# masa-ue/SVDD

Measured on AMD Instinct MI355X. Metric: decoded sequences/sec (whole node), L=200 M=10 128-step SVDD-MC, higher is better.
Workload: dtype f32; 1 GPU; DNA enhancer SVDD-MC, batch=256/GPU, L=200, M=10, 128 steps (BASELINE.json configs[1]); dilated-CNN backbone 3.3M params + ConvGRU value net; global_batch=256, rng=philox

## Files before the change

### include/svdd_hip.h

```cpp
#ifndef SVDD_HIP_H
#define SVDD_HIP_H

#include <stdint.h>

#ifdef __cplusplus
extern "C" {
#endif

#define SVDD_VOCAB 5
#define SVDD_MASK 4
#define SVDD_MAX_M 1024

enum {
  SVDD_OK = 0,
  SVDD_E_ARG = -1,
  SVDD_E_LAUNCH = -2,
  SVDD_E_NODEVICE = -3
};

enum {
  SVDD_LAYOUT_BLV = 0,
  SVDD_LAYOUT_BVL = 1
};

// ... 109 lines not shown
int svdd_gru_set_mode(int mode);

int svdd_epilogue_ln_f32(const float* y, const float* bias, const float* f_prev, const float* tb,
                         const float* gamma, const float* beta, float* f_out, float* hn, int64_t rows,
                         int channels, int act, void* stream);

int svdd_conv1d_cl_f32(const float* x, const float* wpack, float* y, int n, int L, int cin, int cout,
                       int taps, int dilation, const float* bias, const float* f_prev, int act,
                       const float* tb, const float* gamma, const float* beta, float* hn, void* stream);
int svdd_conv1d_set_dynamic(int on);

int svdd_conv_tower_f32(const float* onehot, const float* tiles, const float* bias, float* out, int n, int L,
                        int nlayers, int residual_mask, const int32_t* count, void* stream);

int svdd_set_backbone_packing(int full);

int svdd_set_tower_version(int v);

int svdd_candidate_windows(const uint8_t* cand, const uint8_t* x, int B, int L, int M, int margin, int32_t* win,
                           int32_t* flags, void* stream);
int svdd_conv_tower_windows_f32(const float* onehot, const float* tiles, const float* bias, const int32_t* win,
                                const float* parent_out, float* out, int n, int L, int M, int nlayers,
                                int residual_mask, const int32_t* live_idx, const int32_t* count, void* stream);

int svdd_backbone_cnn_f32(const uint8_t* x, const float* table0, const float* tiles, const float* vec,
                          const float* w2, float* out, int n, int L, int nlayers, const int* dilations,
                          const int32_t* count, const int32_t* row_idx, int out_scatter, void* stream);
int svdd_backbone_cnn_save_f32(const uint8_t* x, const float* table0, const float* tiles, const float* vec, const float* w2,
                               float* out, int n, int L, int nlayers, const int* dilations, float* xhat, float* rstd,
                               unsigned long long* mask, void* stream);
int svdd_backbone_cnn_grad_f32(const float* dlogits, const float* tiles_bwd, const float* gamma, const float* w2,
                               const float* table0, const float* xhat, const float* rstd, const unsigned long long* mask,
                               float* dx, int n, int L, int nlayers, const int* dilations, void* stream);
int svdd_backbone_incr_f32(const uint8_t* x, const float* table0, const float* tiles, const float* vec, const float* w2,
                           float* out, int n, int L, int nlayers, const int* dilations, int lead, float* planes,
                           uint8_t* x_prev, int32_t* items, unsigned long long* stat, int first, int max_item, void* on_stream);
int svdd_backbone_incr2_f32(const uint8_t* x, const float* table0, const float* tiles, const float* vec, const float* w2,
                            float* out, int n, int L, int nlayers, const int* dilations, int lead, float* planes,
                            uint8_t* x_prev, int32_t* items, unsigned long long* stat, int first, int max_item,
                            int32_t* order, int32_t* order_count, void* on_stream);
int svdd_backbone_incr_set_residency(int wg_per_cu);
int svdd_backbone_set_workspace(void* ws, long long bytes);
int svdd_backbone_split_status(int* err);

enum { SVDD_PREC_F32 = 0, SVDD_PREC_F16X3 = 1, SVDD_PREC_BF16X3 = 2, SVDD_PREC_F16 = 3, SVDD_PREC_BF16 = 4 };

int svdd_backbone_cnn_lp(const uint8_t* x, const float* table0, const void* tiles, const float* vec,
                         const float* lscale, const float* w2, float* out, int n, int L, int nlayers,
                         const int* dilations, int prec, const int32_t* count, const int32_t* row_idx, int out_scatter,
                         void* stream);

int svdd_conv_tower_lp(const uint8_t* tok, const void* tiles, const float* bias, const float* inv, void* out,
                       int n, int L, int nlayers, int residual_mask, const int32_t* count, int prec, void* stream);
int svdd_conv_tower_windows_lp(const uint8_t* cand, const void* tiles, const float* bias, const float* inv,
                               const int32_t* win, const void* parent_out, void* out, int n, int L, int M,
                               int nlayers, int residual_mask, const int32_t* live_idx, const int32_t* count,
                               int prec, void* stream);

int svdd_gru_bidir_lp(const float* x, const void* x16, const void* wpack, const float* bpack, const float* inv,
                      float* out, int n, int L, const int32_t* count, int prec, void* stream);

int svdd_value_tail_lp(const float* h_fwd, const float* h_bwd, const void* w1pack, const float* b1,
                       const float* w_eff, const float* b_eff, float inv, float* out, int n, int L, int n_tasks,
                       const int32_t* count, int prec, void* stream);
// ... 69 lines not shown
```

### svdd_amd/_lib.py

```python
import ctypes
import os
import subprocess

_HERE = os.path.dirname(os.path.abspath(__file__))
CSRC = os.path.join(_HERE, "csrc")
SO_PATH = os.environ.get("SVDD_HIP_LIB") or os.path.join(CSRC, "libsvdd_hip.so")
ABI_VERSION = 17

OK, E_ARG, E_LAUNCH, E_NODEVICE = 0, -1, -2, -3
LAYOUT_BLV, LAYOUT_BVL = 0, 1
RNG_REPLAY, RNG_PHILOX = 0, 1
SELECT_ARGMAX, SELECT_MULTINOMIAL = 0, 1
TARGET_MEAN, TARGET_LOGMEANEXP = 0, 1
EVOLVE_GLOBAL, EVOLVE_ROW = 0, 1
ATTR_GRADIENT, ATTR_TIMES_INPUT = 0, 1
PRECISIONS = {"f32": 0, "f16x3": 1, "bf16x3": 2, "f16": 3, "bf16": 4}
MAX_M = 1024

OPT_FORCE_EXACT, OPT_MSPLIT, OPT_SELECT_ONE_ROW, OPT_BACKBONE_LP_VERSION, OPT_TRUNK_GEMM_VERSION = 0, 1, 2, 3, 4
OPT_CAND_ROW_STRIDE, OPT_TRUNK_PLANES_F32, OPT_BACKBONE_SPLIT, OPT_SELECT_BATCHES = 5, 6, 7, 8


class SvddRng(ctypes.Structure):
    _fields_ = [("kind", ctypes.c_int32), ("step", ctypes.c_uint32), ("uniforms", ctypes.c_void_p),
# ... 72 lines not shown
    "svdd_backbone_split_status": (pi32,),
    "svdd_backbone_cnn_save_f32": (vp, vp, vp, vp, vp, vp, i32, i32, i32, pi32, vp, vp, vp, STREAM),
    "svdd_backbone_cnn_grad_f32": (vp, vp, vp, vp, vp, vp, vp, vp, vp, i32, i32, i32, pi32, STREAM),
    "svdd_dps_probs": (vp, vp, i32, i32, vp, STREAM),
    "svdd_dps_probs_bwd": (vp, vp, vp, i32, i32, vp, vp, STREAM),
    "svdd_dps_guided_q": (vp, vp, vp, vp, f32, f32, f32, i32, i32, vp, STREAM),
    "svdd_reward_stem_f32": (vp, vp, vp, vp, i32, i32, i32, STREAM),
    "svdd_reward_stem_bwd_f32": (vp, vp, vp, i32, i32, i32, STREAM),
    "svdd_conv1d_cl_gated_f32": (vp, vp, vp, i32, i32, i32, i32, i32, i32, vp, vp, STREAM),
    "svdd_reward_tail_grad_f32": (vp, vp, vp, vp, vp, vp, vp, f32, i32, i32, vp, vp, STREAM),
    "svdd_sum_gate_f32": (vp, vp, vp, vp, i64, STREAM),
    "svdd_gru_bidir_train2_f32": (vp, vp, vp, vp, vp, vp, i32, i32, STREAM),
    "svdd_gru_bidir_bwd2_f32": (vp, vp, vp, vp, vp, vp, vp, i32, i32, STREAM),
    "svdd_classifier_propose": (vp, i32, vp, vp, f32, f32, f32, i32, i32, RNG, vp, vp, vp, STREAM),
    "svdd_elbo_mask": (vp, i32, i32, i32, f64, RNG, vp, vp, vp, vp, vp, vp, STREAM),
    "svdd_elbo_nll": (vp, i32, vp, vp, vp, i32, i32, i32, vp, vp, vp, vp, STREAM),
    "svdd_refine_remask": (vp, vp, vp, vp, vp, f32, i32, i32, RNG, vp, vp, vp, vp, vp, vp, vp),
    "svdd_value_target": (vp, vp, i32, i32, i32, i32, f32, vp, vp, vp, vp),
    "svdd_ism_mutants": (vp, vp, vp, i32, i32, i32, vp, vp, vp, vp),
    "svdd_ism_fold": (vp, vp, vp, vp, vp, vp, i32, i32, i32, i32, i32, vp, vp, vp, vp, vp),
    "svdd_evolve_apply": (vp, vp, vp, i32, i32, i32, vp, vp, vp, vp, vp, vp, vp, vp, vp, vp, vp, vp),
    "svdd_attr_path": (vp, vp, i32, vp, i32, i32, i32, i32, i32, i32, vp, vp, vp),
    "svdd_attr_fold": (vp, f32, vp, vp, vp, i32, i32, i32, i32, i32, i32, i32, vp, vp, vp, vp),
}
EXPORTS = tuple(SIGNATURES)


def build(force=False):
    import glob
    srcs = sorted(glob.glob(os.path.join(CSRC, "*.hip")) + glob.glob(os.path.join(CSRC, "*.h")) + [os.path.join(CSRC, "Makefile")])
    srcs.append(os.path.join(os.path.dirname(_HERE), "include", "svdd_hip.h"))
    if os.environ.get("SVDD_HIP_LIB"):
        return SO_PATH
    stale = not os.path.exists(SO_PATH) or os.path.getmtime(SO_PATH) < max(os.path.getmtime(f) for f in srcs)
    if force or stale:
        subprocess.check_call(["make", "-C", CSRC, "-B", "-j", str(min(8, os.cpu_count() or 1))])
    return SO_PATH


_lib = None


def lib():
    global _lib
    if _lib is not None:
        return _lib
# ... 112 lines not shown
```

### svdd_amd/csrc/svdd_nets.hip

```cpp
#include "svdd_host.h"

namespace {

typedef float f32x4 __attribute__((ext_vector_type(4)));

__device__ __forceinline__ float wave_sum(float v) {
#pragma unroll
  for (int off = 32; off > 0; off >>= 1) v += __shfl_xor(v, off, 64);
  return v;
}


constexpr int H = 64;
constexpr int HPAD = H + 4;

__device__ __forceinline__ float sigmoid_fast(float a) {
  return __builtin_amdgcn_rcpf(1.0f + __builtin_amdgcn_exp2f(-1.44269504088896f * a));
}
__device__ __forceinline__ float tanh_fast(float a) {
  return 1.0f - 2.0f * __builtin_amdgcn_rcpf(1.0f + __builtin_amdgcn_exp2f(2.88539008177793f * a));
}

template <bool BOTH>
__global__ __launch_bounds__(BOTH ? 512 : 256) void gru_bidir_kernel(const float* __restrict__ x, const float* __restrict__ wpack,
// ... 1163 lines not shown

__global__ __launch_bounds__(256) void candidate_windows_kernel(const uint8_t* __restrict__ cand, const uint8_t* __restrict__ x,
                                                               int n, int L, int M, int margin, int* __restrict__ win,
                                                               int* __restrict__ flags) {
  const int c = blockIdx.x * 4 + (threadIdx.x >> 6);
  if (c >= n) return;
  const int lane = threadIdx.x & 63;
  const uint8_t* cp = cand + (size_t)c * L;
  const uint8_t* xp = x + (size_t)(c / M) * L;
  int lo = 1 << 30, hi = -1;
  for (int l = lane; l < L; l += 64)
    if (cp[l] != xp[l]) { lo = min(lo, l); hi = max(hi, l); }
#pragma unroll
  for (int off = 32; off > 0; off >>= 1) { lo = min(lo, __shfl_xor(lo, off, 64)); hi = max(hi, __shfl_xor(hi, off, 64)); }
  if (lane == 0) {
    int w0 = 0, w1 = 0;
    if (hi >= 0) {
      w0 = max(0, lo - margin) & ~15;
      w1 = min((L + 15) & ~15, (hi + margin + 1 + 15) & ~15);
    }
    win[2 * c] = w0; win[2 * c + 1] = w1;
    if (flags) flags[c] = (w1 - w0) >> 4;
  }
}


struct BackboneArgs {
  const uint8_t* x;
  const float* table0;
  const float* tiles;
  const float* vec;
  const float* w2;
  float* out;
  int n, L, spt, nl;
  int dil[BB_MAXL];
  const int* count;
  const int* row_idx;
  int out_scatter;
  int auto_spt, ncu;
  SvddTilePlan plan;
  float* planes;
  int planes_P;
};

struct BackboneSave {
  float* xhat;
// ... 435 lines not shown
    const float* wv = a.w2 + v * BB_C;
    float sm = a.w2[5 * BB_C + v];
#pragma unroll 8
    for (int k = 0; k < BB_C; ++k) sm += hr[k] * wv[k];
    const int64_t sq = (a.row_idx && a.out_scatter) ? (int64_t)a.row_idx[seq0 + q] : (int64_t)(seq0 + q);
    a.out[(sq * L + pos) * 5 + v] = sm;
  }
}
#undef BB_OWN

constexpr int SEG_SLOTS = 7;

struct BackboneSegArgs {
  const uint8_t* x;
  const float* table0;
  const float* tiles;
  const float* vec;
  float* planes;
  const int* items;
  int n, L, layer;
  const int* order;
  const int* order_count;
  int order_stride;
};

template <int SLOTS = SEG_SLOTS>
__global__ __launch_bounds__(256) void backbone_worklist_kernel(const uint8_t* __restrict__ x, uint8_t* __restrict__ x_prev, int n,
                                                                int L, int P, int max_item, int* __restrict__ items,
                                                                unsigned long long* __restrict__ stat) {
  const int row = blockIdx.x * 4 + (threadIdx.x >> 6);
  if (row >= n) return;
  const int lane = threadIdx.x & 63;
  const uint8_t* xn = x + (size_t)row * L;
  uint8_t* xp = x_prev + (size_t)row * L;
  int changed = 0;
  for (int q = 0; q < 4; ++q) {
    const int l = lane + 64 * q;
    if (l < L && xn[l] != xp[l]) { changed |= 1 << q; xp[l] = xn[l]; }
  }
  int mine = 0;
  for (int k = 1; k <= P; ++k) {
    const int reach = 4 + 4 * k;
    int m = 0;
    for (int q = 0; q < 4; ++q)
      if (changed >> q & 1) {
        const int l = lane + 64 * q;
        const int tlo = max(0, l - reach) >> 4, thi = min(L - 1, l + reach) >> 4;
        m |= ((2 << thi) - 1) & ~((1 << tlo) - 1);
      }
#pragma unroll
    for (int off = 32; off > 0; off >>= 1) m |= __shfl_xor(m, off, 64);
    if (lane == k - 1) mine = m;
  }
  if (lane >= P) return;
  int* it = items + ((size_t)lane * n + row) * SLOTS;
  int cnt = 0;
  for (int t = 0; t < TW_RT;) {
    if (!(mine >> t & 1)) { ++t; continue; }
    int len = 1;
    while (len < max_item && t + len < TW_RT && (mine >> (t + len) & 1)) ++len;
    it[cnt++] = t | len << 8;
// ... 72 lines not shown
    if ((int)blockIdx.x >= a.order_count[a.layer - 1]) return;
    const unsigned ent = (unsigned)__builtin_amdgcn_readfirstlane(a.order[(size_t)(a.layer - 1) * a.order_stride + blockIdx.x]);
    item = (int)(ent & 0xFFFFu);
    seq = (int)(ent >> 16);
  } else {
    item = __builtin_amdgcn_readfirstlane(a.items[(size_t)(a.layer - 1) * a.n * SEG_SLOTS + blockIdx.x]);
    seq = blockIdx.x / SEG_SLOTS;
  }
  const int nown = min(item >> 8, NC);
  if (nown == 0) return;
  const int t0 = item & 255;
  const int tid = threadIdx.x, lane = tid & 63;
  const int cg = __builtin_amdgcn_readfirstlane(tid >> 6);
  const int j = lane & 15, g = lane >> 4;
  const int col0 = 32 * cg + j;
  const int L = a.L;
  const int r0 = 16 * (t0 - 1);
  const size_t pl_stride = (size_t)a.n * TW_ROWS * BB_C;
  float* pl0 = a.planes + (size_t)seq * TW_ROWS * BB_C;
  const int cl = a.layer - 1;
#define SEG_LIVE(S) ((S) <= nown + 1)

  f32x4 f[NS][2], acc[NS][2];
  if (a.layer == 1) {
    for (int e = tid; e < ROWS + 8; e += 256) {
      const int p = r0 - 4 + e;
      toks[e] = (p >= 0 && p < L) ? (int)a.x[(size_t)seq * L + p] : -1;
    }
    __syncthreads();
#pragma unroll
    for (int ct = 0; ct < 2; ++ct) {
      const int col = col0 + 16 * ct;
      const float b0 = a.vec[col];
#pragma unroll
      for (int s = 0; s < NS; ++s) {
        if (!SEG_LIVE(s)) continue;
#pragma unroll
        for (int e = 0; e < 4; ++e) {
          const int ri = 16 * s + 4 * g + e, row = r0 + ri;
          float v = b0;
#pragma unroll
          for (int t = 0; t < 9; ++t) {
            const int tk = toks[ri + t];
            if (tk >= 0) v += a.table0[(t * 5 + tk) * BB_C + col];
          }
          f[s][ct][e] = (row >= 0 && row < L) ? fmaxf(v, 0.0f) : 0.0f;
        }
      }
    }
  } else {
    const float* src = pl0 + (size_t)(a.layer - 2) * pl_stride;
#pragma unroll
    for (int s = 0; s < NS; ++s) {
      if (!SEG_LIVE(s)) continue;
#pragma unroll
      for (int ct = 0; ct < 2; ++ct)
#pragma unroll
        for (int e = 0; e < 4; ++e) {
          const int row = r0 + 16 * s + 4 * g + e;
          f[s][ct][e] = (row >= 0 && row < L) ? src[row * BB_C + col0 + 16 * ct] : 0.0f;
        }
    }
  }

  const float* vl = a.vec + (size_t)(cl + 1) * 4 * BB_C;
  {
    const float tb0 = vl[BB_C + col0], tb1 = vl[BB_C + col0 + 16];
#pragma unroll
    for (int s = 0; s < NS; ++s) {
      if (!SEG_LIVE(s)) continue;
#pragma unroll
      for (int e = 0; e < 4; ++e) {
        const float sm = group16_sum((f[s][0][e] + tb0) + (f[s][1][e] + tb1));
        if (j == 0) psum[cg * ROWS + 16 * s + 4 * g + e] = sm;
// ... 1062 lines not shown
  }
  const bool spt1 = !a.auto_spt && a.plan.s2 == 1 && (a.plan.n1 == 0 || a.plan.s1 == 1);
  return svdd_launch_timed(ev, spt1 ? backbone_kernel<true> : backbone_kernel<false>, dim3(nwg), dim3(512), lds, stream, a, BackboneSave{});
}

extern "C" int svdd_backbone_incr_f32(const uint8_t* x, const float* table0, const float* tiles, const float* vec, const float* w2,
                                      float* out, int n, int L, int nlayers, const int* dilations, int lead, float* planes,
                                      uint8_t* x_prev, int32_t* items, unsigned long long* stat, int first, int max_item,
                                      void* stream) {
  if (!x || !table0 || !tiles || !vec || !w2 || !out || !dilations || !planes || !x_prev || !items || n <= 0 || L <= TW_ROWS / 2 ||
      L > TW_ROWS || nlayers <= 0 || nlayers > BB_MAXL || lead < 2 || lead > nlayers || (max_item != 2 && max_item != 4))
    return SVDD_E_ARG;
  for (int i = 0; i < lead; ++i) if (dilations[i] != 1) return SVDD_E_ARG;
  BackboneArgs a;
  if (!backbone_args(a, x, table0, tiles, vec, w2, out, n, L, 1, nlayers, dilations)) return SVDD_E_ARG;
  a.planes = planes; a.planes_P = lead;
  const SvddLds lds = svdd_lds_raised(backbone_lds_bytes(nlayers, 3));
  SvddSpan span(SVDD_SLOT_BACKBONE);
  if (first) {
    if (hipMemcpyAsync(x_prev, x, (size_t)n * L, hipMemcpyDeviceToDevice, (hipStream_t)stream) != hipSuccess) return SVDD_E_LAUNCH;
    return svdd_launch_timed(span.all(), backbone_kernel<true, false, 1>, dim3((unsigned)n), dim3(512), lds, stream, a, BackboneSave{});
  }
  if (svdd_launch_timed(span.first(), backbone_worklist_kernel<>, dim3((unsigned)((n + 3) / 4)), dim3(256), 0, stream, x, x_prev, n, L, lead,
                        max_item, items, stat) != SVDD_OK)
    return SVDD_E_LAUNCH;
  BackboneSegArgs sa{x, table0, tiles, vec, planes, items, n, L, 0, nullptr, nullptr, 0};
  const int rows = 16 * (max_item + 2);
  const size_t slds = sizeof(float) * ((size_t)rows * BB_AP + 5 * (size_t)rows + rows + 8);
  const dim3 sgrid((unsigned)n * SEG_SLOTS);
  void (*seg)(BackboneSegArgs) = max_item == 4 ? backbone_seg_kernel<4> : backbone_seg_kernel<2>;
  svdd_raise_lds_limit(seg, slds);
  for (int k = 1; k <= lead; ++k) {
    sa.layer = k;
    if (svdd_launch(seg, sgrid, dim3(256), slds, stream, sa) != SVDD_OK) return SVDD_E_LAUNCH;
  }
  return svdd_launch_timed(span.last(), backbone_kernel<true, false, 2>, dim3((unsigned)n), dim3(512), lds, stream, a, BackboneSave{});
}

constexpr int INCR_DEFAULT_RESIDENCY = 0;
constexpr size_t CU_LDS_BYTES = 160 * 1024;
static int g_incr_residency = INCR_DEFAULT_RESIDENCY;

extern "C" int svdd_backbone_incr_set_residency(int wg_per_cu) {
  if (wg_per_cu < 0 || wg_per_cu > 8) return SVDD_E_ARG;
  g_incr_residency = wg_per_cu;
  return SVDD_OK;
}

extern "C" int svdd_backbone_incr2_f32(const uint8_t* x, const float* table0, const float* tiles, const float* vec, const float* w2,
                                       float* out, int n, int L, int nlayers, const int* dilations, int lead, float* planes,
                                       uint8_t* x_prev, int32_t* items, unsigned long long* stat, int first, int max_item,
                                       int32_t* order, int32_t* order_count, void* stream) {
  if (!x || !table0 || !tiles || !vec || !w2 || !out || !dilations || !planes || !x_prev || !items || !order || !order_count ||
      n <= 0 || n > 65536 || L <= TW_ROWS / 2 || L > TW_ROWS || nlayers <= 0 || nlayers > BB_MAXL || lead < 2 || lead > nlayers ||
      (max_item != 1 && max_item != 2 && max_item != 4))
    return SVDD_E_ARG;
  for (int i = 0; i < lead; ++i) if (dilations[i] != 1) return SVDD_E_ARG;
  BackboneArgs a;
  if (!backbone_args(a, x, table0, tiles, vec, w2, out, n, L, 1, nlayers, dilations)) return SVDD_E_ARG;
  a.planes = planes; a.planes_P = lead;
  const SvddLds lds = svdd_lds_raised(backbone_lds_bytes(nlayers, 3));
  SvddSpan span(SVDD_SLOT_BACKBONE);
  if (first) {
    if (hipMemcpyAsync(x_prev, x, (size_t)n * L, hipMemcpyDeviceToDevice, (hipStream_t)stream) != hipSuccess) return SVDD_E_LAUNCH;
    return svdd_launch_timed(span.all(), backbone_kernel<true, false, 1>, dim3((unsigned)n), dim3(512), lds, stream, a, BackboneSave{});
  }
  const int slots = max_item == 1 ? TW_RT : SEG_SLOTS;
  if (svdd_launch_timed(span.first(), max_item == 1 ? backbone_worklist_kernel<TW_RT> : backbone_worklist_kernel<SEG_SLOTS>,
                        dim3((unsigned)((n + 3) / 4)), dim3(256), 0, stream, x, x_prev, n, L, lead, max_item, items, stat) != SVDD_OK)
    return SVDD_E_LAUNCH;
  if (svdd_launch(max_item == 1 ? backbone_order_kernel<TW_RT> : backbone_order_kernel<SEG_SLOTS>, dim3((unsigned)lead), dim3(256), 0, stream,
                  items, n, order, order_count) != SVDD_OK)
    return SVDD_E_LAUNCH;
  BackboneSegArgs sa{x, table0, tiles, vec, planes, items, n, L, 0, order, order_count, n * slots};
  const int rows = 16 * (max_item + 2);
  size_t slds = sizeof(float) * ((size_t)rows * BB_AP + 5 * (size_t)rows + rows + 8);
  if (g_incr_residency > 0) {
    const size_t pad = (CU_LDS_BYTES / (size_t)(g_incr_residency + 1) / 1024 + 1) * 1024;
    if (pad > slds) slds = pad;
  }
  const dim3 sgrid((unsigned)(n * slots));
  void (*seg)(BackboneSegArgs) = max_item == 4 ? backbone_seg_kernel<4, true> : max_item == 2 ? backbone_seg_kernel<2, true>
                                                                                                : backbone_seg_kernel<1, true>;
  svdd_raise_lds_limit(seg, slds);
  for (int k = 1; k <= lead; ++k) {
    sa.layer = k;
    if (svdd_launch(seg, sgrid, dim3(256), slds, stream, sa) != SVDD_OK) return SVDD_E_LAUNCH;
  }
  return svdd_launch_timed(span.last(), backbone_kernel<true, false, 2>, dim3((unsigned)n), dim3(512), lds, stream, a, BackboneSave{});
}

typedef decltype(&value_tail_kernel<1>) ValueTailKernel;

extern "C" int svdd_value_tail_f32(const float* h_fwd, const float* h_bwd, const float* w1pack, const float* b1,
                                   const float* w_eff, const float* b_eff, float* out, int n, int L, int n_tasks,
                                   const int32_t* count, void* stream) {
  if (!h_fwd || !h_bwd || !w1pack || !b1 || !w_eff || !b_eff || !out || n <= 0 || L <= 0 || n_tasks < 1 || n_tasks > 4)
    return SVDD_E_ARG;
  ValueTailKernel kern;
  switch (n_tasks) {
    case 1: kern = value_tail_kernel<1>; break;
    case 2: kern = value_tail_kernel<2>; break;
    case 3: kern = value_tail_kernel<3>; break;
    default: kern = value_tail_kernel<4>; break;
  }
  SvddSpan span(SVDD_SLOT_VALUE_TAIL);
  return svdd_launch_timed(span.all(), kern, dim3((unsigned)((n + 3) / 4)), dim3(256), 0, stream, h_fwd, h_bwd, w1pack, b1, w_eff, b_eff, out,
                           n, L, count);
}

extern "C" int svdd_candidate_windows(const uint8_t* cand, const uint8_t* x, int B, int L, int M, int margin, int32_t* win,
                                      int32_t* flags, void* stream) {
  if (!cand || !x || !win || B <= 0 || L <= 0 || M <= 0 || margin < 0) return SVDD_E_ARG;
  const int n = B * M;
  return svdd_launch(candidate_windows_kernel, dim3((unsigned)((n + 3) / 4)), dim3(256), 0, stream, cand, x, n, L, M, margin, win, flags);
}

extern "C" int svdd_conv_tower_windows_f32(const float* onehot, const float* tiles, const float* bias, const int32_t* win,
                                           const float* parent_out, float* out, int n, int L, int M, int nlayers,
                                           int residual_mask, const int32_t* live_idx, const int32_t* count, void* stream) {
  if (!onehot || !tiles || !bias || !win || !parent_out || !out || n <= 0 || M <= 0 || (n % M && !live_idx) || L <= TW_ROWS / 2 ||
      L > TW_ROWS || nlayers != 5)
    return SVDD_E_ARG;
  TowerWinArgs wa{TowerArgs{onehot, tiles, bias, out, n, L, 1, nlayers, residual_mask, nullptr}, win, parent_out, M, live_idx, count};
  void (*kern)(TowerWinArgs) = conv_tower_win_kernel;
  if (g_tower_ver != 1) kern = g_tower_ver == 2 ? conv_tower2_kernel<true, true, 2> : conv_tower2_kernel<true, true, 1>;
  SvddSpan span(SVDD_SLOT_CONV_TOWER);
  return svdd_launch_timed(span.all(), kern, dim3((unsigned)n), dim3(512), svdd_lds_raised(tower2_lds_bytes()), stream, wa);
}
```

### svdd_amd/fused.py

```python
import ctypes
import math

import torch
import torch.nn.functional as F
from torch import nn

from . import _lib
from .backbone import CNNModel
from .value_nets import ConvGRUTrunk, ConvHead


def _cl(w):
    return w.detach().unsqueeze(2).contiguous(memory_format=torch.channels_last)


def pack_gru(gru):
    H = gru.hidden_size
    assert H == 64 and gru.input_size == 64 and gru.bidirectional and gru.num_layers == 1 and gru.bias
    packs, biases = [], []
    for sfx in ("", "_reverse"):
        w_ih = getattr(gru, "weight_ih_l0" + sfx).detach().float()
        w_hh = getattr(gru, "weight_hh_l0" + sfx).detach().float()
        b_ih = getattr(gru, "bias_ih_l0" + sfx).detach().float()
        b_hh = getattr(gru, "bias_hh_l0" + sfx).detach().float()
# ... 291 lines not shown
    if err.value:
        raise _lib.SvddError("svdd_backbone_cnn_f32: a workgroup of a small-batch (several workgroups per sequence) launch waited in vain "
                             "for its partners — something else occupied the CUs (another process or stream on this GPU). The logits "
                             "of that launch are invalid. Run with svdd_set_option(SVDD_OPT_BACKBONE_SPLIT, 1) when the GPU is shared.")


def backbone_cnn(tokens, pk, count=None, out=None, row_idx=None, scatter=False):
    global _bb_split_used
    assert tokens.is_cuda and tokens.dtype == torch.uint8 and tokens.is_contiguous()
    n, L = tokens.shape
    if 104 < L <= 208 and count is None and row_idx is None and (n <= BB_SPLIT_MAX_SEQ or 0 < n % 256 <= BB_SPLIT_MAX_SEQ):
        _backbone_split_workspace(tokens.device)
        _bb_split_used = True
    if out is None:
        out = torch.empty((n, L, 5), dtype=torch.float32, device=tokens.device)
    dil = (ctypes.c_int * len(pk["dil"]))(*pk["dil"])
    _lib.call("svdd_backbone_cnn_f32", tokens, pk["table0"], pk["tiles"], pk["vec"], pk["w2"], out, n, L, len(pk["dil"]), dil, count,
              row_idx, int(scatter))
    return out


INCR_MAX_ITEM = 2
INCR_ORDERED = True
INCR_RESIDENCY = 0
INCR_SLOTS = 13


def set_incr_residency(r):
    global INCR_RESIDENCY
    _lib.call("svdd_backbone_incr_set_residency", int(r))
    INCR_RESIDENCY = int(r)


def leading_dilation1(dil):
    n = 0
    while n < len(dil) and dil[n] == 1:
        n += 1
    return n


class IncrementalStem:

    def __init__(self, n, L, lead, dev):
        self.n, self.L, self.lead = n, L, lead
        self.planes = torch.empty((lead, n, 208, 128), dtype=torch.float32, device=dev)
        self.x_prev = torch.empty((n, L), dtype=torch.uint8, device=dev)
        self.items = torch.zeros((lead, n, INCR_SLOTS), dtype=torch.int32, device=dev)
        self.order = torch.zeros((lead, n * INCR_SLOTS), dtype=torch.int32, device=dev)
        self.order_count = torch.zeros(lead, dtype=torch.int32, device=dev)
        self.stat = torch.zeros(1, dtype=torch.int64, device=dev)
        self.valid = False
        self.forwards = 0


def backbone_cnn_incremental(tokens, pk, st, out=None, max_item=None):
    assert tokens.is_cuda and tokens.dtype == torch.uint8 and tokens.is_contiguous() and tuple(tokens.shape) == (st.n, st.L)
    n, L = tokens.shape
    if out is None:
        out = torch.empty((n, L, 5), dtype=torch.float32, device=tokens.device)
    dil = (ctypes.c_int * len(pk["dil"]))(*pk["dil"])
    first = not st.valid
    stream = ctypes.c_void_p(torch.cuda.current_stream().cuda_stream)
    if INCR_ORDERED:
        _lib.call("svdd_backbone_incr2_f32", tokens, pk["table0"], pk["tiles"], pk["vec"], pk["w2"], out, n, L, len(pk["dil"]), dil,
                  st.lead, st.planes, st.x_prev, st.items, st.stat, int(first), int(max_item or INCR_MAX_ITEM), st.order,
                  st.order_count, stream)
    else:
        _lib.call("svdd_backbone_incr_f32", tokens, pk["table0"], pk["tiles"], pk["vec"], pk["w2"], out, n, L, len(pk["dil"]), dil,
                  st.lead, st.planes, st.x_prev, st.items, st.stat, int(first), int(max_item or INCR_MAX_ITEM), stream)
    st.valid = True
    st.forwards += 0 if first else 1
    return out


LP_DTYPES = {"f16x3": (torch.float16, 2), "bf16x3": (torch.bfloat16, 2), "f16": (torch.float16, 1), "bf16": (torch.bfloat16, 1)}


def _pow2_floor(v):
    return 2.0 ** math.floor(math.log2(v))


def _split16(w, dtype, parts):
    hi = w.to(dtype)
    if parts == 1:
        return hi.unsqueeze(-1)
    lo = (w - hi.float()).to(dtype)
    return torch.stack([hi, lo], dim=-1)


def pack_backbone_lp(cnn, precision):
    dtype, parts = LP_DTYPES[precision]
    pk = pack_backbone(cnn)
    H, nl = 128, len(cnn.convs)
# ... 107 lines not shown
        out = torch.empty((2, n, L, 64), dtype=torch.float32, device=x_nlc.device)
    _lib.call("svdd_gru_bidir_lp", None if split else x_nlc, x_nlc if split else None, wpack, bpack, inv, out, n, L, count, prec)
    return out


def value_tail_lp(h, w1pack, b1f, w_eff, b_eff, inv, prec, count=None, out=None):
    _, n, L, _ = h.shape
    T = w_eff.shape[1]
    if out is None:
        out = torch.empty((n, T), dtype=torch.float32, device=h.device)
    assert out.is_contiguous() and out.shape == (n, T) and out.dtype == torch.float32
    _lib.call("svdd_value_tail_lp", h[0], h[1], w1pack, b1f, w_eff, b_eff, float(inv), out, n, L, T, count, prec)
    return out


TOWER_WINDOW_MARGIN = 27


def candidate_windows(cand, x, margin=TOWER_WINDOW_MARGIN, flags=None):
    assert cand.is_cuda and cand.dtype == torch.uint8 and cand.is_contiguous() and x.dtype == torch.uint8 and x.is_contiguous()
    B, M, L = cand.shape
    win = torch.empty((B * M, 2), dtype=torch.int32, device=cand.device)
    _lib.call("svdd_candidate_windows", cand, x, B, L, M, margin, win, flags)
    return win


def conv_tower_windows(onehot, win, parent_out, M, tiles, bias, residual_mask, live_idx=None, count=None, out=None):
    assert onehot.is_cuda and onehot.dtype == torch.float32 and onehot.is_contiguous() and onehot.shape[2] == 4
    n, L, _ = onehot.shape
    assert parent_out.is_contiguous() and parent_out.shape == (n // M, L, 64) and win.shape == (n, 2)
    if out is None:
        out = torch.empty((n, L, 64), dtype=torch.float32, device=onehot.device)
    else:
        assert live_idx is not None and count is not None and out.is_contiguous() and out.shape[1:] == (L, 64)
        n = out.shape[0]
    _lib.call("svdd_conv_tower_windows_f32", onehot, tiles, bias, win, parent_out, out, n, L, M, bias.shape[0] - 1, int(residual_mask),
              live_idx, count)
    return out


def epilogue_ln(y, bias=None, f_prev=None, tb=None, gamma=None, beta=None, act=ACT_RELU_THEN_ADD, want_norm=True,
                want_sum=True):
    C = bias.numel() if bias is not None else gamma.numel()
    rows = y.numel() // C
    f = torch.empty_like(y) if want_sum else None
    hn = torch.empty_like(y) if want_norm else None
# ... 149 lines not shown
        if self.gru_off_chain:
            _lib.call("svdd_gru_bidir_bwd2_f32", gout, out, save, gru_bwd, gates, fs[-1], g, n, L)
        else:
            dxd = torch.empty_like(out)
            _lib.call("svdd_gru_bidir_bwd_f32", gout, out, save, gru_bwd, dxd, n, L)
            _lib.call("svdd_sum_gate_f32", dxd[0], dxd[1], fs[-1], g, n * L * 64)
        bufs = [gout[1], dxg[0]]
        for k in range(len(packs_t) - 1, -1, -1):
            y = bufs[k & 1]
            _lib.call("svdd_conv1d_cl_gated_f32", g, packs_t[k], y, n, L, 64, 64, 5, 1, g if self.residual[k] else None, fs[k])
            g = y
        dx = torch.empty((n, L, 4), dtype=torch.float32, device=dev)
        _lib.call("svdd_reward_stem_bwd_f32", g, w_stem, dx, n, L, self._stem_w_raw.shape[2])
        if self.keep_grad_pass:
            self.last_grad_pass = {"fs": fs, "out": out, "g_tail": gout[0], "grad": dx}
        return dx

    def kernels_ok(self, L):
        return self.use_fused_tower and self.tower_ok and self.use_fused_tail and self.tail_ok and L <= 208

    def candidate_scores_compact(self, onehot, cand, x, ws):
        from . import ops
        B, M, L = cand.shape
        win = candidate_windows(cand, x, flags=ws.flags)
        split = self._gru_split(B * M) if (self.precision == "f32" and getattr(ws, "late", False)) else 0
        if split:
            ops.compact_by_key(ws.flags, ws.live_idx, ws.slot, ws.count3, split=split)
        else:
            (ops.compact_by_key if self.sort_live_by_window else ops.compact_flags)(ws.flags, ws.live_idx, ws.slot, ws.count)
        if getattr(ws, "n_win_rows", None) is not None:
            ws.n_win_rows += (win[:, 1] - win[:, 0]).sum()
        lp = self.precision != "f32"
        if ws.parent_out is None or ws.parent_out_lp != self.precision:
            xp = x[:1].contiguous() if getattr(ws, "prior_rows_identical", False) else x
            if lp:
                pk = self._lp_pack()
                po = conv_tower_lp(xp, pk["tiles"], self.tw_bias, pk["tinv"], self.tw_resmask, pk["prec"])
            else:
                po = conv_tower(ops.transform_samples(xp), self.tw_tiles, self.tw_bias, self.tw_resmask)
            ws.parent_out = po if xp is x else po.expand(B, *po.shape[1:]).contiguous()
            ws.prior_rows_identical = False
            ws.parent_out_lp = self.precision
        if lp:
            pk = self._lp_pack()
            ws.seq = conv_tower_windows_lp(cand, win, ws.parent_out, pk["tiles"], self.tw_bias, pk["tinv"], self.tw_resmask,
                                           pk["prec"], live_idx=ws.live_idx, count=ws.count)
            return self._after_tower_lp(ws.seq, pk, ws.count)[:, :, 0]
        if split:
            return self._windows_gru_tail_split(onehot, win, ws, B * M, L, M, split)
        ws.seq = conv_tower_windows(onehot, win, ws.parent_out, M, self.tw_tiles, self.tw_bias, self.tw_resmask,
                                    live_idx=ws.live_idx, count=ws.count)
        return self._after_tower(ws.seq, B * M, L, ws.count)[:, :, 0]
# ... 244 lines not shown
```

Measured before the change: 768.8 sequences/s.

## Fuse candidate windows with live-list compaction and cache incremental backbone layer-0 plane

Adds a single-launch kernel that computes candidate edit windows and then, using a last-block ticket, builds the window-keyed compacted live list in the same launch. This replaces the separate windows and compact_by_key launches. It also adds an incremental backbone variant that stores a layer-0 embedding plane and recomputes only the rows near changed tokens inside the worklist kernel. The segment kernels then read that plane instead of rebuilding layer 1 from tokens. The cost is an extra plane buffer of size n×208×128 floats, a serial tail in the last block of the compaction, and a dependence on correct atomic ticket resets between calls.

```diff
diff --git a/include/svdd_hip.h b/include/svdd_hip.h
--- a/include/svdd_hip.h
+++ b/include/svdd_hip.h
@@ -155,6 +155,8 @@
 int svdd_conv_tower_windows_f32(const float* onehot, const float* tiles, const float* bias, const int32_t* win,
                                 const float* parent_out, float* out, int n, int L, int M, int nlayers,
                                 int residual_mask, const int32_t* live_idx, const int32_t* count, void* stream);
+int svdd_candidate_live_list(const uint8_t* cand, const uint8_t* x, int B, int L, int M, int margin, int split, int32_t* win,
+                             int32_t* flags, int32_t* live_idx, int32_t* slot, int32_t* count, uint32_t* ticket, void* on_stream);
 
 int svdd_backbone_cnn_f32(const uint8_t* x, const float* table0, const float* tiles, const float* vec,
                           const float* w2, float* out, int n, int L, int nlayers, const int* dilations,
@@ -173,6 +175,10 @@
                             uint8_t* x_prev, int32_t* items, unsigned long long* stat, int first, int max_item,
                             int32_t* order, int32_t* order_count, void* on_stream);
 int svdd_backbone_incr_set_residency(int wg_per_cu);
+int svdd_backbone_incr3_f32(const uint8_t* x, const float* table0, const float* tiles, const float* vec, const float* w2,
+                            float* out, int n, int L, int nlayers, const int* dilations, int lead, float* planes,
+                            uint8_t* x_prev, int32_t* items, unsigned long long* stat, int first, int max_item,
+                            int32_t* order, int32_t* order_count, void* on_stream);
 int svdd_backbone_set_workspace(void* ws, long long bytes);
 int svdd_backbone_split_status(int* err);
 
diff --git a/svdd_amd/_lib.py b/svdd_amd/_lib.py
--- a/svdd_amd/_lib.py
+++ b/svdd_amd/_lib.py
@@ -118,6 +118,8 @@
     "svdd_evolve_apply": (vp, vp, vp, i32, i32, i32, vp, vp, vp, vp, vp, vp, vp, vp, vp, vp, vp, vp),
     "svdd_attr_path": (vp, vp, i32, vp, i32, i32, i32, i32, i32, i32, vp, vp, vp),
     "svdd_attr_fold": (vp, f32, vp, vp, vp, i32, i32, i32, i32, i32, i32, i32, vp, vp, vp, vp),
+    "svdd_backbone_incr3_f32": (vp, vp, vp, vp, vp, vp, i32, i32, i32, pi32, i32, vp, vp, vp, vp, i32, i32, vp, vp, vp),
+    "svdd_candidate_live_list": (vp, vp, i32, i32, i32, i32, i32, vp, vp, vp, vp, vp, vp, vp),
 }
 EXPORTS = tuple(SIGNATURES)
 
diff --git a/svdd_amd/csrc/svdd_nets.hip b/svdd_amd/csrc/svdd_nets.hip
--- a/svdd_amd/csrc/svdd_nets.hip
+++ b/svdd_amd/csrc/svdd_nets.hip
@@ -1209,6 +1209,104 @@
     win[2 * c] = w0; win[2 * c + 1] = w1;
     if (flags) flags[c] = (w1 - w0) >> 4;
   }
+}
+
+constexpr int LIVE_THREADS = 1024;
+__global__ __launch_bounds__(LIVE_THREADS) void candidate_live_list_kernel(const uint8_t* __restrict__ cand, const uint8_t* __restrict__ x,
+                                                                           int n, int L, int M, int margin, int* __restrict__ win,
+                                                                           int* flags, int* __restrict__ live_idx, int* __restrict__ slot,
+                                                                           int* __restrict__ count, int split, unsigned* ticket) {
+  __shared__ unsigned wave_tot[LIVE_THREADS / 64][8];
+  __shared__ unsigned block_tot[8];
+  __shared__ int is_last;
+  const int tid = threadIdx.x, lane = tid & 63, w = tid >> 6;
+  const int c = blockIdx.x * (LIVE_THREADS / 64) + w;
+  if (c < n) {
+    const uint8_t* cp = cand + (size_t)c * L;
+    const uint8_t* xp = x + (size_t)(c / M) * L;
+    int lo = 1 << 30, hi = -1;
+    for (int l = lane; l < L; l += 64)
+      if (cp[l] != xp[l]) { lo = min(lo, l); hi = max(hi, l); }
+#pragma unroll
+    for (int off = 32; off > 0; off >>= 1) { lo = min(lo, __shfl_xor(lo, off, 64)); hi = max(hi, __shfl_xor(hi, off, 64)); }
+    if (lane == 0) {
+      int w0 = 0, w1 = 0;
+      if (hi >= 0) {
+        w0 = max(0, lo - margin) & ~15;
+        w1 = min((L + 15) & ~15, (hi + margin + 1 + 15) & ~15);
+      }
+      win[2 * c] = w0; win[2 * c + 1] = w1;
+      flags[c] = (w1 - w0) >> 4;
+    }
+  }
+  asm volatile("s_waitcnt vmcnt(0)" ::: "memory");
+  __syncthreads();
+  if (tid == 0) {
+    __threadfence();
+    asm volatile("s_waitcnt vmcnt(0)" ::: "memory");
+    const unsigned t = __hip_atomic_fetch_add(ticket, 1u, __ATOMIC_RELAXED, __HIP_MEMORY_SCOPE_AGENT);
+    const int last = t == gridDim.x - 1;
+    if (last) {
+      __threadfence();
+      asm volatile("s_waitcnt vmcnt(0)" ::: "memory");
+      __hip_atomic_store(ticket, 0u, __ATOMIC_RELAXED, __HIP_MEMORY_SCOPE_AGENT);
+    }
+    is_last = last;
+  }
+  __syncthreads();
+  if (!is_last) return;
+
+  const int chunk = (n + LIVE_THREADS - 1) / LIVE_THREADS;
+  const int i0 = min(tid * chunk, n), i1 = min(i0 + chunk, n);
+#define LIVE_KEY(I) min(max(__hip_atomic_load(flags + (I), __ATOMIC_RELAXED, __HIP_MEMORY_SCOPE_AGENT), 0), 15)
+  unsigned cnt[8] = {0, 0, 0, 0, 0, 0, 0, 0};
+#pragma unroll 1
+  for (int i = i0; i < i1; ++i) {
+    const int k = LIVE_KEY(i);
+#pragma unroll
+    for (int q = 0; q < 8; ++q) cnt[q] += (k >> 1) == q ? 1u << (16 * (k & 1)) : 0u;
+  }
+  unsigned pre[8];
+#pragma unroll
+  for (int q = 0; q < 8; ++q) {
+    unsigned v = cnt[q];
+#pragma unroll
+    for (int off = 1; off < 64; off <<= 1) { const unsigned u = __shfl_up(v, off, 64); if (lane >= off) v += u; }
+    pre[q] = v - cnt[q];
+    if (lane == 63) wave_tot[w][q] = v;
+  }
+  __syncthreads();
+  if (tid < 8) {
+    unsigned t = 0;
+    for (int ww = 0; ww < LIVE_THREADS / 64; ++ww) { const unsigned v = wave_tot[ww][tid]; wave_tot[ww][tid] = t; t += v; }
+    block_tot[tid] = t;
+  }
+  __syncthreads();
+  unsigned tot[8];
+#pragma unroll
+  for (int q = 0; q < 8; ++q) { pre[q] += wave_tot[w][q]; tot[q] = block_tot[q]; }
+  int at[16];
+  int run = 0;
+#pragma unroll
+  for (int k = 15; k >= 1; --k) {
+    at[k] = run + (int)(pre[k >> 1] >> (16 * (k & 1)) & 0xFFFFu);
+    run += (int)(tot[k >> 1] >> (16 * (k & 1)) & 0xFFFFu);
+  }
+  if (tid == 0) {
+    count[0] = run;
+    if (split > 0) { count[1] = min(run, split); count[2] = max(run - split, 0); }
+  }
+#pragma unroll 1
+  for (int i = i0; i < i1; ++i) {
+    const int k = LIVE_KEY(i);
+    int o = -1;
+#pragma unroll
+    for (int kk = 1; kk < 16; ++kk)
+      if (k == kk) o = at[kk]++;
+    if (o >= 0) live_idx[o] = i;
+    slot[i] = o;
+  }
+#undef LIVE_KEY
 }
 
 
@@ -1690,21 +1788,96 @@
   const int* order;
   const int* order_count;
   int order_stride;
+  const float* plane0;
 };
 
-template <int SLOTS = SEG_SLOTS>
+template <int SLOTS = SEG_SLOTS, bool P0 = false>
 __global__ __launch_bounds__(256) void backbone_worklist_kernel(const uint8_t* __restrict__ x, uint8_t* __restrict__ x_prev, int n,
                                                                 int L, int P, int max_item, int* __restrict__ items,
-                                                                unsigned long long* __restrict__ stat) {
-  const int row = blockIdx.x * 4 + (threadIdx.x >> 6);
+                                                                unsigned long long* __restrict__ stat,
+                                                                const float* __restrict__ table0 = nullptr,
+                                                                const float* __restrict__ b_first = nullptr,
+                                                                float* __restrict__ plane0 = nullptr, int all = 0) {
+  const int row = P0 ? (int)blockIdx.x : (int)(blockIdx.x * 4 + (threadIdx.x >> 6));
+  const int wv = P0 ? (int)(threadIdx.x >> 6) : 0;
   if (row >= n) return;
   const int lane = threadIdx.x & 63;
   const uint8_t* xn = x + (size_t)row * L;
   uint8_t* xp = x_prev + (size_t)row * L;
   int changed = 0;
+  unsigned tok4 = 0;
   for (int q = 0; q < 4; ++q) {
     const int l = lane + 64 * q;
-    if (l < L && xn[l] != xp[l]) { changed |= 1 << q; xp[l] = xn[l]; }
+    if (l < L) {
+      const uint8_t tn = xn[l];
+      if (P0) tok4 |= (unsigned)tn << (8 * q);
+      if (tn != xp[l]) { changed |= 1 << q; if (!P0) xp[l] = tn; }
+    }
+  }
+  if constexpr (P0) {
+    __syncthreads();
+    if (wv == 0)
+      for (int q = 0; q < 4; ++q)
+        if (changed >> q & 1) xp[lane + 64 * q] = (uint8_t)(tok4 >> (8 * q));
+    unsigned long long need[4];
+    {
+      unsigned long long ch[4];
+      for (int q = 0; q < 4; ++q) ch[q] = all ? ~0ull : __ballot(changed >> q & 1);
+      for (int q = 0; q < 4; ++q) {
+        unsigned long long m = ch[q];
+        for (int d = 1; d <= 4; ++d) {
+          m |= ch[q] << d | ch[q] >> d;
+          if (q > 0) m |= ch[q - 1] >> (64 - d);
+          if (q < 3) m |= ch[q + 1] << (64 - d);
+        }
+        const int left = L - 64 * q;
+        need[q] = left >= 64 ? m : left <= 0 ? 0ull : m & ((1ull << left) - 1ull);
+      }
+    }
+    float* prow = plane0 + (size_t)row * TW_ROWS * BB_C;
+    const int qw = lane >> 4, c8 = 8 * (lane & 15);
+    const float4 bias0 = *reinterpret_cast<const float4*>(b_first + c8), bias1 = *reinterpret_cast<const float4*>(b_first + c8 + 4);
+    unsigned long long cur = need[0];
+    int wd = 0;
+    auto take = [&]() -> int {
+      while (cur == 0ull && wd < 3) { ++wd; cur = wd == 1 ? need[1] : wd == 2 ? need[2] : need[3]; }
+      if (cur == 0ull) return -1;
+      const int b = __ffsll((long long)cur) - 1;
+      cur &= cur - 1ull;
+      return 64 * wd + b;
+    };
+    for (int pass = 0;; ++pass) {
+      const int ra = take(), rb = take(), rc = take(), rd = take();
+      if (ra < 0) break;
+      if ((pass & 3) != wv) continue;
+      const int r = qw == 0 ? ra : qw == 1 ? rb : qw == 2 ? rc : rd;
+      float4 tv[9][2];
+      bool in[9];
+#pragma unroll
+      for (int t = 0; t < 9; ++t) {
+        const int p = r + t - 4;
+        in[t] = r >= 0 && p >= 0 && p < L;
+        const unsigned w = (unsigned)__shfl((int)tok4, in[t] ? p & 63 : 0, 64);
+        const int tk = in[t] ? (int)(w >> (8 * (p >> 6)) & 255u) : 0;
+        const float* src = table0 + (size_t)(t * 5 + tk) * BB_C + c8;
+        tv[t][0] = *reinterpret_cast<const float4*>(src);
+        tv[t][1] = *reinterpret_cast<const float4*>(src + 4);
+      }
+      float4 v0 = bias0, v1 = bias1;
+#pragma unroll
+      for (int t = 0; t < 9; ++t) {
+        v0.x = in[t] ? v0.x + tv[t][0].x : v0.x; v0.y = in[t] ? v0.y + tv[t][0].y : v0.y;
+        v0.z = in[t] ? v0.z + tv[t][0].z : v0.z; v0.w = in[t] ? v0.w + tv[t][0].w : v0.w;
+        v1.x = in[t] ? v1.x + tv[t][1].x : v1.x; v1.y = in[t] ? v1.y + tv[t][1].y : v1.y;
+        v1.z = in[t] ? v1.z + tv[t][1].z : v1.z; v1.w = in[t] ? v1.w + tv[t][1].w : v1.w;
+      }
+      if (r >= 0) {
+        float* dst = prow + (size_t)r * BB_C + c8;
+        *reinterpret_cast<float4*>(dst) = make_float4(fmaxf(v0.x, 0.0f), fmaxf(v0.y, 0.0f), fmaxf(v0.z, 0.0f), fmaxf(v0.w, 0.0f));
+        *reinterpret_cast<float4*>(dst + 4) = make_float4(fmaxf(v1.x, 0.0f), fmaxf(v1.y, 0.0f), fmaxf(v1.z, 0.0f), fmaxf(v1.w, 0.0f));
+      }
+    }
+    if (all || wv != 0) return;
   }
   int mine = 0;
   for (int k = 1; k <= P; ++k) {
@@ -1823,7 +1996,7 @@
 #define SEG_LIVE(S) ((S) <= nown + 1)
 
   f32x4 f[NS][2], acc[NS][2];
-  if (a.layer == 1) {
+  if (a.layer == 1 && !a.plane0) {
     for (int e = tid; e < ROWS + 8; e += 256) {
       const int p = r0 - 4 + e;
       toks[e] = (p >= 0 && p < L) ? (int)a.x[(size_t)seq * L + p] : -1;
@@ -1850,7 +2023,7 @@
       }
     }
   } else {
-    const float* src = pl0 + (size_t)(a.layer - 2) * pl_stride;
+    const float* src = a.layer == 1 ? a.plane0 + (size_t)seq * TW_ROWS * BB_C : pl0 + (size_t)(a.layer - 2) * pl_stride;
 #pragma unroll
     for (int s = 0; s < NS; ++s) {
       if (!SEG_LIVE(s)) continue;
@@ -2959,9 +3132,9 @@
     return svdd_launch_timed(span.all(), backbone_kernel<true, false, 1>, dim3((unsigned)n), dim3(512), lds, stream, a, BackboneSave{});
   }
   if (svdd_launch_timed(span.first(), backbone_worklist_kernel<>, dim3((unsigned)((n + 3) / 4)), dim3(256), 0, stream, x, x_prev, n, L, lead,
-                        max_item, items, stat) != SVDD_OK)
+                        max_item, items, stat, (const float*)nullptr, (const float*)nullptr, (float*)nullptr, 0) != SVDD_OK)
     return SVDD_E_LAUNCH;
-  BackboneSegArgs sa{x, table0, tiles, vec, planes, items, n, L, 0, nullptr, nullptr, 0};
+  BackboneSegArgs sa{x, table0, tiles, vec, planes, items, n, L, 0, nullptr, nullptr, 0, nullptr};
   const int rows = 16 * (max_item + 2);
   const size_t slds = sizeof(float) * ((size_t)rows * BB_AP + 5 * (size_t)rows + rows + 8);
   const dim3 sgrid((unsigned)n * SEG_SLOTS);
@@ -2984,10 +3157,10 @@
   return SVDD_OK;
 }
 
-extern "C" int svdd_backbone_incr2_f32(const uint8_t* x, const float* table0, const float* tiles, const float* vec, const float* w2,
-                                       float* out, int n, int L, int nlayers, const int* dilations, int lead, float* planes,
-                                       uint8_t* x_prev, int32_t* items, unsigned long long* stat, int first, int max_item,
-                                       int32_t* order, int32_t* order_count, void* stream) {
+static int backbone_incr_ordered(const uint8_t* x, const float* table0, const float* tiles, const float* vec, const float* w2,
+                                 float* out, int n, int L, int nlayers, const int* dilations, int lead, float* planes,
+                                 uint8_t* x_prev, int32_t* items, unsigned long long* stat, int first, int max_item,
+                                 int32_t* order, int32_t* order_count, void* stream, bool p0) {
   if (!x || !table0 || !tiles || !vec || !w2 || !out || !dilations || !planes || !x_prev || !items || !order || !order_count ||
       n <= 0 || n > 65536 || L <= TW_ROWS / 2 || L > TW_ROWS || nlayers <= 0 || nlayers > BB_MAXL || lead < 2 || lead > nlayers ||
       (max_item != 1 && max_item != 2 && max_item != 4))
@@ -2995,21 +3168,33 @@
   for (int i = 0; i < lead; ++i) if (dilations[i] != 1) return SVDD_E_ARG;
   BackboneArgs a;
   if (!backbone_args(a, x, table0, tiles, vec, w2, out, n, L, 1, nlayers, dilations)) return SVDD_E_ARG;
-  a.planes = planes; a.planes_P = lead;
+  float* const plane1 = p0 ? planes + (size_t)n * TW_ROWS * BB_C : planes;
+  a.planes = plane1; a.planes_P = lead;
   const SvddLds lds = svdd_lds_raised(backbone_lds_bytes(nlayers, 3));
   SvddSpan span(SVDD_SLOT_BACKBONE);
+  const dim3 wgrid((unsigned)((n + 3) / 4));
   if (first) {
     if (hipMemcpyAsync(x_prev, x, (size_t)n * L, hipMemcpyDeviceToDevice, (hipStream_t)stream) != hipSuccess) return SVDD_E_LAUNCH;
-    return svdd_launch_timed(span.all(), backbone_kernel<true, false, 1>, dim3((unsigned)n), dim3(512), lds, stream, a, BackboneSave{});
+    if (!p0)
+      return svdd_launch_timed(span.all(), backbone_kernel<true, false, 1>, dim3((unsigned)n), dim3(512), lds, stream, a, BackboneSave{});
+    if (svdd_launch_timed(span.first(), backbone_worklist_kernel<SEG_SLOTS, true>, dim3((unsigned)n), dim3(256), 0, stream, x, x_prev, n, L, lead, max_item,
+                          items, stat, table0, vec, planes, 1) != SVDD_OK)
+      return SVDD_E_LAUNCH;
+    return svdd_launch_timed(span.last(), backbone_kernel<true, false, 1>, dim3((unsigned)n), dim3(512), lds, stream, a, BackboneSave{});
   }
   const int slots = max_item == 1 ? TW_RT : SEG_SLOTS;
-  if (svdd_launch_timed(span.first(), max_item == 1 ? backbone_worklist_kernel<TW_RT> : backbone_worklist_kernel<SEG_SLOTS>,
-                        dim3((unsigned)((n + 3) / 4)), dim3(256), 0, stream, x, x_prev, n, L, lead, max_item, items, stat) != SVDD_OK)
+  if (p0) {
+    if (svdd_launch_timed(span.first(), max_item == 1 ? backbone_worklist_kernel<TW_RT, true> : backbone_worklist_kernel<SEG_SLOTS, true>,
+                          dim3((unsigned)n), dim3(256), 0, stream, x, x_prev, n, L, lead, max_item, items, stat, table0, vec, planes, 0) != SVDD_OK)
+      return SVDD_E_LAUNCH;
+  } else if (svdd_launch_timed(span.first(), max_item == 1 ? backbone_worklist_kernel<TW_RT> : backbone_worklist_kernel<SEG_SLOTS>, wgrid,
+                               dim3(256), 0, stream, x, x_prev, n, L, lead, max_item, items, stat, (const float*)nullptr,
+                               (const float*)nullptr, (float*)nullptr, 0) != SVDD_OK)
     return SVDD_E_LAUNCH;
   if (svdd_launch(max_item == 1 ? backbone_order_kernel<TW_RT> : backbone_order_kernel<SEG_SLOTS>, dim3((unsigned)lead), dim3(256), 0, stream,
                   items, n, order, order_count) != SVDD_OK)
     return SVDD_E_LAUNCH;
-  BackboneSegArgs sa{x, table0, tiles, vec, planes, items, n, L, 0, order, order_count, n * slots};
+  BackboneSegArgs sa{x, table0, tiles, vec, plane1, items, n, L, 0, order, order_count, n * slots, p0 ? planes : nullptr};
   const int rows = 16 * (max_item + 2);
   size_t slds = sizeof(float) * ((size_t)rows * BB_AP + 5 * (size_t)rows + rows + 8);
   if (g_incr_residency > 0) {
@@ -3025,6 +3210,22 @@
     if (svdd_launch(seg, sgrid, dim3(256), slds, stream, sa) != SVDD_OK) return SVDD_E_LAUNCH;
   }
   return svdd_launch_timed(span.last(), backbone_kernel<true, false, 2>, dim3((unsigned)n), dim3(512), lds, stream, a, BackboneSave{});
+}
+
+extern "C" int svdd_backbone_incr2_f32(const uint8_t* x, const float* table0, const float* tiles, const float* vec, const float* w2,
+                                       float* out, int n, int L, int nlayers, const int* dilations, int lead, float* planes,
+                                       uint8_t* x_prev, int32_t* items, unsigned long long* stat, int first, int max_item,
+                                       int32_t* order, int32_t* order_count, void* stream) {
+  return backbone_incr_ordered(x, table0, tiles, vec, w2, out, n, L, nlayers, dilations, lead, planes, x_prev, items, stat, first, max_item,
+                               order, order_count, stream, false);
+}
+
+extern "C" int svdd_backbone_incr3_f32(const uint8_t* x, const float* table0, const float* tiles, const float* vec, const float* w2,
+                                       float* out, int n, int L, int nlayers, const int* dilations, int lead, float* planes,
+                                       uint8_t* x_prev, int32_t* items, unsigned long long* stat, int first, int max_item,
+                                       int32_t* order, int32_t* order_count, void* stream) {
+  return backbone_incr_ordered(x, table0, tiles, vec, w2, out, n, L, nlayers, dilations, lead, planes, x_prev, items, stat, first, max_item,
+                               order, order_count, stream, true);
 }
 
 typedef decltype(&value_tail_kernel<1>) ValueTailKernel;
@@ -3053,6 +3254,16 @@
   return svdd_launch(candidate_windows_kernel, dim3((unsigned)((n + 3) / 4)), dim3(256), 0, stream, cand, x, n, L, M, margin, win, flags);
 }
 
+extern "C" int svdd_candidate_live_list(const uint8_t* cand, const uint8_t* x, int B, int L, int M, int margin, int split, int32_t* win,
+                                        int32_t* flags, int32_t* live_idx, int32_t* slot, int32_t* count, uint32_t* ticket, void* stream) {
+  if (!cand || !x || !win || !flags || !live_idx || !slot || !count || !ticket || B <= 0 || L <= 0 || M <= 0 || margin < 0 || split < 0 ||
+      (int64_t)B * M > 65535)
+    return SVDD_E_ARG;
+  const int n = B * M, per = LIVE_THREADS / 64;
+  return svdd_launch(candidate_live_list_kernel, dim3((unsigned)((n + per - 1) / per)), dim3(LIVE_THREADS), 0, stream, cand, x, n, L, M, margin,
+                     win, flags, live_idx, slot, count, split, ticket);
+}
+
 extern "C" int svdd_conv_tower_windows_f32(const float* onehot, const float* tiles, const float* bias, const int32_t* win,
                                            const float* parent_out, float* out, int n, int L, int M, int nlayers,
                                            int residual_mask, const int32_t* live_idx, const int32_t* count, void* stream) {
diff --git a/svdd_amd/fused.py b/svdd_amd/fused.py
--- a/svdd_amd/fused.py
+++ b/svdd_amd/fused.py
@@ -337,6 +337,7 @@
 
 INCR_MAX_ITEM = 2
 INCR_ORDERED = True
+INCR_PLANE0 = True
 INCR_RESIDENCY = 0
 INCR_SLOTS = 13
 
@@ -358,7 +359,9 @@
 
     def __init__(self, n, L, lead, dev):
         self.n, self.L, self.lead = n, L, lead
-        self.planes = torch.empty((lead, n, 208, 128), dtype=torch.float32, device=dev)
+        self.planes0 = torch.empty((lead + 1, n, 208, 128), dtype=torch.float32, device=dev)
+        self.planes = self.planes0[1:]
+        self.plane0_valid = False
         self.x_prev = torch.empty((n, L), dtype=torch.uint8, device=dev)
         self.items = torch.zeros((lead, n, INCR_SLOTS), dtype=torch.int32, device=dev)
         self.order = torch.zeros((lead, n * INCR_SLOTS), dtype=torch.int32, device=dev)
@@ -374,16 +377,21 @@
     if out is None:
         out = torch.empty((n, L, 5), dtype=torch.float32, device=tokens.device)
     dil = (ctypes.c_int * len(pk["dil"]))(*pk["dil"])
-    first = not st.valid
+    plane0 = INCR_ORDERED and INCR_PLANE0
+    first = not st.valid or (plane0 and not st.plane0_valid)
     stream = ctypes.c_void_p(torch.cuda.current_stream().cuda_stream)
-    if INCR_ORDERED:
+    if plane0:
+        _lib.call("svdd_backbone_incr3_f32", tokens, pk["table0"], pk["tiles"], pk["vec"], pk["w2"], out, n, L, len(pk["dil"]), dil,
+                  st.lead, st.planes0, st.x_prev, st.items, st.stat, int(first), int(max_item or INCR_MAX_ITEM), st.order,
+                  st.order_count, stream)
+    elif INCR_ORDERED:
         _lib.call("svdd_backbone_incr2_f32", tokens, pk["table0"], pk["tiles"], pk["vec"], pk["w2"], out, n, L, len(pk["dil"]), dil,
                   st.lead, st.planes, st.x_prev, st.items, st.stat, int(first), int(max_item or INCR_MAX_ITEM), st.order,
                   st.order_count, stream)
     else:
         _lib.call("svdd_backbone_incr_f32", tokens, pk["table0"], pk["tiles"], pk["vec"], pk["w2"], out, n, L, len(pk["dil"]), dil,
                   st.lead, st.planes, st.x_prev, st.items, st.stat, int(first), int(max_item or INCR_MAX_ITEM), stream)
-    st.valid = True
+    st.valid, st.plane0_valid = True, plane0
     st.forwards += 0 if first else 1
     return out
 
@@ -537,6 +545,18 @@
     B, M, L = cand.shape
     win = torch.empty((B * M, 2), dtype=torch.int32, device=cand.device)
     _lib.call("svdd_candidate_windows", cand, x, B, L, M, margin, win, flags)
+    return win
+
+
+LIVE_LIST_ONE_LAUNCH = True
+
+
+def candidate_live_list(cand, x, flags, live_idx, slot, count, ticket, split=0, margin=TOWER_WINDOW_MARGIN):
+    assert cand.is_cuda and cand.dtype == torch.uint8 and cand.is_contiguous() and x.dtype == torch.uint8 and x.is_contiguous()
+    B, M, L = cand.shape
+    win = torch.empty((B * M, 2), dtype=torch.int32, device=cand.device)
+    stream = ctypes.c_void_p(torch.cuda.current_stream().cuda_stream)
+    _lib.call("svdd_candidate_live_list", cand, x, B, L, M, margin, int(split), win, flags, live_idx, slot, count, ticket, stream)
     return win
 
 
@@ -732,12 +752,17 @@
     def candidate_scores_compact(self, onehot, cand, x, ws):
         from . import ops
         B, M, L = cand.shape
-        win = candidate_windows(cand, x, flags=ws.flags)
         split = self._gru_split(B * M) if (self.precision == "f32" and getattr(ws, "late", False)) else 0
-        if split:
-            ops.compact_by_key(ws.flags, ws.live_idx, ws.slot, ws.count3, split=split)
+        if LIVE_LIST_ONE_LAUNCH and (split or self.sort_live_by_window) and B * M <= 65535:
+            if getattr(ws, "live_ticket", None) is None:
+                ws.live_ticket = torch.zeros(1, dtype=torch.int32, device=cand.device)
+            win = candidate_live_list(cand, x, ws.flags, ws.live_idx, ws.slot, ws.count3 if split else ws.count, ws.live_ticket, split=split)
         else:
-            (ops.compact_by_key if self.sort_live_by_window else ops.compact_flags)(ws.flags, ws.live_idx, ws.slot, ws.count)
+            win = candidate_windows(cand, x, flags=ws.flags)
+            if split:
+                ops.compact_by_key(ws.flags, ws.live_idx, ws.slot, ws.count3, split=split)
+            else:
+                (ops.compact_by_key if self.sort_live_by_window else ops.compact_flags)(ws.flags, ws.live_idx, ws.slot, ws.count)
         if getattr(ws, "n_win_rows", None) is not None:
             ws.n_win_rows += (win[:, 1] - win[:, 0]).sum()
         lp = self.precision != "f32"
```

Result: no change. 775.0 sequences/s, median of 6 (+0.8%).
